# ml-unito/PartitionedLS.jl

Measured on AMD Instinct MI355X. Metric: sign-pattern NNLS solves/sec (whole node); fp64 obj gap vs ref, higher is better.
Workload: dtype f64

## Files before the change

### include/partls.h

```cpp
#ifndef PARTLS_H
#define PARTLS_H
#include <stdint.h>
#ifdef __cplusplus
extern "C" {
#endif

typedef enum {
    PARTLS_OK = 0,
    PARTLS_ERR_BAD_ARG = 1,
    PARTLS_ERR_BAD_PARTITION = 2,
    PARTLS_ERR_NONFINITE = 3,
    PARTLS_ERR_NO_DEVICE = 4,
    PARTLS_ERR_HIP = 5,
    PARTLS_ERR_NOT_CONVERGED = 6,
    PARTLS_ERR_UNSUPPORTED = 7,
    PARTLS_ERR_STATE = 8,
    PARTLS_ERR_ILL_CONDITIONED = 9
} partls_status;

#define PARTLS_OPT_FAITHFUL_INTERCEPT 1u
#define PARTLS_OPT_GENERIC_KERNEL     2u
#define PARTLS_OPT_RESCUE_CAPPED      4u

typedef struct partls_ctx partls_ctx;
// ... 105 lines not shown
partls_status partls_frontier_create(int n_groups, int rank, int world, int64_t batch, partls_frontier **out);
void          partls_frontier_destroy(partls_frontier *f);
partls_status partls_frontier_next(partls_frontier *f, int64_t *total, int64_t *mine, uint64_t *pat, uint64_t *free_groups,
                                   int32_t *src_slot, int32_t *per_rank);
partls_status partls_frontier_ingest(partls_frontier *f, const double *lb, const int32_t *branch, const int32_t *dst_slot,
                                     int32_t *dead, int64_t dead_capacity, int64_t *ndead);
partls_status partls_frontier_result(const partls_frontier *f, double *mu, uint64_t *pat, uint64_t *free_groups, int64_t *nodes);
partls_status partls_bnb_search(partls_ctx *ctx, int64_t max_nodes, double *mu, uint64_t *pat, uint64_t *free_groups, int64_t *nodes);

partls_status partls_predict(partls_ctx *ctx, const double *X, int64_t N, int64_t M, int64_t ldX,
                             const int64_t *P, int64_t K, int64_t ldP, const double *alpha, const double *beta, double t,
                             double *yhat);
partls_status partls_predict_device(partls_ctx *ctx, const double *dX, int64_t N, int64_t M, int64_t ldX,
                                    const int64_t *P, int64_t K, int64_t ldP, const double *alpha, const double *beta,
                                    double t, double *dyhat);


#define PARTLS_PREDICT_MANY_CHUNK 16
#define PARTLS_PREDICT_MANY_MAX_B 4096
#define PARTLS_PREDICT_MANY_BYTES (64ULL << 20)
partls_status partls_predict_many(partls_ctx *ctx, const double *X, int64_t N, int64_t M, int64_t ldX, int x_on_device,
                                  const int64_t *P, int64_t K, int64_t ldP, int64_t B, const double *alpha, const double *beta,
                                  const double *t, double *yhat, int64_t ldY, int64_t nr, const int64_t *ranks, double *stats,
                                  double *mean);

partls_status partls_synth_truth(uint64_t seed, int64_t D, int64_t K, int64_t *P, double *wstar);
partls_status partls_synth_device(partls_ctx *ctx, uint64_t seed, int64_t N, int64_t D, const double *wstar,
                                  double *dX, double *dy);

typedef enum {
    PARTLS_T_GRAM = 0,
    PARTLS_T_PREP = 1,
    PARTLS_T_SWEEP = 2,
    PARTLS_T_FINISH = 3,
    PARTLS_T_CALIB = 4,
    PARTLS_T_OOB = 5,
    PARTLS_T_RESCUE = 6,
    PARTLS_T_COUNT = 7
} partls_timer;
partls_status partls_get_timing(const partls_ctx *ctx, partls_timer which, double *ms);
partls_status partls_get_upload(const partls_ctx *ctx, double *ms, double *bytes);
partls_status partls_get_pivots(const partls_ctx *ctx, int64_t *pivots);
partls_status partls_get_vetoes(const partls_ctx *ctx, int64_t *vetoes);
partls_status partls_get_rescue_stats(const partls_ctx *ctx, int64_t *rescued, int64_t *pivots, int64_t *failed);
partls_status partls_get_blocks(const partls_ctx *ctx, int64_t *blocks);
partls_status partls_get_kkt_violation(const partls_ctx *ctx, double *violation, double *min_pivot);
typedef enum {
    PARTLS_ROUTE_REG_256 = 1,
    PARTLS_ROUTE_REG_512 = 2,
    PARTLS_ROUTE_DEFERRED = 3,
    PARTLS_ROUTE_EAGER = 4
} partls_route;
partls_status partls_get_sweep_route(const partls_ctx *ctx, int *kernel, int *tiles);
partls_status partls_get_near_ties(const partls_ctx *ctx, int64_t *evaluated);
partls_status partls_get_gram(const partls_ctx *ctx, double *G_aug);

#include "partls_f32.h"
#include "partls_f32_more.h"

#ifdef __cplusplus
}
#endif
#endif
```

### partitionedls.jl_amd/_lib.py

```python
import ctypes as C
import os
import subprocess

_HERE = os.path.dirname(os.path.abspath(__file__))
SO_PATH = os.environ.get("PARTLS_LIB") or os.path.join(_HERE, "libpartls_hip.so")
CSRC = os.path.join(_HERE, "csrc")

OK, ERR_BAD_ARG, ERR_BAD_PARTITION, ERR_NONFINITE, ERR_NO_DEVICE, ERR_HIP, ERR_NOT_CONVERGED, ERR_UNSUPPORTED, ERR_STATE, ERR_ILL_CONDITIONED = range(10)
OPT_FAITHFUL_INTERCEPT = 1
OPT_GENERIC_KERNEL = 2
OPT_RESCUE_CAPPED = 4
T_GRAM, T_PREP, T_SWEEP, T_FINISH, T_CALIB, T_OOB, T_RESCUE = range(7)
ROUTE_REG_256, ROUTE_REG_512, ROUTE_DEFERRED, ROUTE_EAGER = range(1, 5)
PREDICT_MANY_CHUNK, PREDICT_MANY_MAX_B, PREDICT_MANY_BYTES = 16, 4096, 64 << 20
OPT_TOP_MAX_K = 4096

_dp = C.POINTER(C.c_double)
_ip = C.POINTER(C.c_int64)
_i64 = C.c_int64

SYMBOLS = [
    ("partls_version", C.c_int, []),
    ("partls_last_error", C.c_char_p, []),
    ("partls_device_count", C.c_int, []),
# ... 21 lines not shown
    ("partls_opt_merge_candidates", C.c_int, [C.c_void_p, _i64, _dp, _ip, _dp, _ip]),
    ("partls_opt_pattern", C.c_int, [C.c_void_p, _i64, _dp, _dp]),
    ("partls_opt_models", C.c_int, [C.c_void_p, _i64, _i64, _ip, _dp, _dp, _i64, _dp, _i64, _dp, _i64, _dp, _ip, _ip]),
    ("partls_opt_top", C.c_int, [C.c_void_p, _i64, _i64, _i64, _ip, _dp, _dp, _i64, _dp, _i64, _dp, _i64, _dp, _ip, _ip, _ip]),
    ("partls_opt_top_select", C.c_int, [C.c_void_p, _dp, _i64, _i64, _i64, _ip, _ip, _dp, _ip]),
    ("partls_cv_opt", C.c_int, [C.c_void_p, C.c_void_p, _i64, _i64, _i64, C.c_void_p, C.c_int, C.c_void_p, _i64, _i64, _ip, _i64,
                                _dp, _i64, C.c_uint32, _dp, _i64, _dp, _i64, _dp, _dp, _ip, _dp, C.POINTER(C.c_int32)]),
    ("partls_cv_opt_weighted", C.c_int, [C.c_void_p, C.c_void_p, _i64, _i64, _i64, C.c_void_p, C.c_void_p, C.c_int, C.c_void_p, _i64,
                                         _i64, _ip, _i64, _dp, _i64, C.c_uint32, _dp, _i64, _dp, _i64, _dp, _dp, _ip, _dp,
                                         C.POINTER(C.c_int32)]),
    ("partls_opt_weightings", C.c_int, [C.c_void_p, C.c_void_p, _i64, _i64, _i64, C.c_void_p, C.c_int, C.c_void_p, _i64, _i64,
                                        C.c_void_p, _i64, _i64, C.c_double, C.c_uint32, _dp, _i64, _dp, _i64, _dp, _dp, _ip, _dp, _ip,
                                        C.POINTER(C.c_int32)]),
    ("partls_opt_num_patterns", _i64, [C.c_void_p]),
    ("partls_opt_bit_order", C.c_int, [C.c_void_p, _ip, _dp]),
    ("partls_fit_alt", C.c_int, [C.c_void_p, C.c_void_p, _i64, _i64, _i64, C.c_void_p, C.c_void_p, _i64, _i64, C.c_double,
                                 C.c_double, _i64, _dp, _dp, _dp, _dp, _dp, _dp, _ip]),
    ("partls_fit_bnb", C.c_int, [C.c_void_p, C.c_void_p, _i64, _i64, _i64, C.c_void_p, C.c_void_p, _i64, _i64, C.c_double,
                                 _dp, _dp, _dp, _dp, _ip]),
    ("partls_alt_prepared", C.c_int, [C.c_void_p, C.c_double, _i64, _dp, _dp, _dp, _dp, _dp, _dp, _ip]),
    ("partls_bnb_prepared", C.c_int, [C.c_void_p, _dp, _dp, _dp, _dp, _ip]),
    ("partls_alt_multistart", C.c_int, [C.c_void_p, C.c_double, _i64, _i64, _dp, _i64, _dp, _i64, _dp, _dp, _dp, _dp, _ip, _ip,
                                        _dp, _i64, _dp, _i64, _dp, _dp, _ip, C.POINTER(C.c_int32)]),
    ("partls_cv_alt", C.c_int, [C.c_void_p, C.c_void_p, _i64, _i64, _i64, C.c_void_p, C.c_void_p, C.c_int, C.c_void_p, _i64, _i64, _ip,
                                _i64, _dp, _i64, C.c_uint32, C.c_double, _i64, _i64, _dp, _i64, _dp, _i64,
                                _dp, _i64, _dp, _i64, _dp, _dp, _ip, _ip, _dp, C.POINTER(C.c_int32), _dp, _ip, C.POINTER(C.c_int32)]),
    ("partls_bnb_bound", C.c_int, [C.c_void_p, _i64, C.POINTER(C.c_uint64), C.POINTER(C.c_uint64), _dp, C.POINTER(C.c_int32)]),
    ("partls_bnb_snap_begin", C.c_int, [C.c_void_p]),
    ("partls_bnb_bound_snap", C.c_int, [C.c_void_p, _i64, C.POINTER(C.c_uint64), C.POINTER(C.c_uint64), C.POINTER(C.c_int32),
                                        C.POINTER(C.c_int32), _dp, C.POINTER(C.c_int32)]),
    ("partls_bnb_snap_release", C.c_int, [C.c_void_p, _i64, C.POINTER(C.c_int32)]),
    ("partls_frontier_create", C.c_int, [C.c_int, C.c_int, C.c_int, _i64, C.POINTER(C.c_void_p)]),
    ("partls_frontier_destroy", None, [C.c_void_p]),
    ("partls_frontier_next", C.c_int, [C.c_void_p, _ip, _ip, C.POINTER(C.c_uint64), C.POINTER(C.c_uint64), C.POINTER(C.c_int32),
                                       C.POINTER(C.c_int32)]),
    ("partls_frontier_ingest", C.c_int, [C.c_void_p, _dp, C.POINTER(C.c_int32), C.POINTER(C.c_int32), C.POINTER(C.c_int32), _i64, _ip]),
    ("partls_frontier_result", C.c_int, [C.c_void_p, _dp, C.POINTER(C.c_uint64), C.POINTER(C.c_uint64), _ip]),
    ("partls_bnb_search", C.c_int, [C.c_void_p, _i64, _dp, C.POINTER(C.c_uint64), C.POINTER(C.c_uint64), _ip]),
    ("partls_bnb_leaf", C.c_int, [C.c_void_p, C.c_uint64, C.c_uint64, _dp, _dp, _dp, _dp]),
    ("partls_predict", C.c_int, [C.c_void_p, C.c_void_p, _i64, _i64, _i64, C.c_void_p, _i64, _i64, _dp, _dp, C.c_double, _dp]),
    ("partls_predict_device", C.c_int, [C.c_void_p, C.c_void_p, _i64, _i64, _i64, C.c_void_p, _i64, _i64, _dp, _dp, C.c_double,
                                        C.c_void_p]),
    ("partls_predict_many", C.c_int, [C.c_void_p, C.c_void_p, _i64, _i64, _i64, C.c_int, C.c_void_p, _i64, _i64, _i64, _dp, _dp, _dp,
                                      C.c_void_p, _i64, _i64, _ip, C.c_void_p, C.c_void_p]),
    ("partls_synth_truth", C.c_int, [C.c_uint64, _i64, _i64, _ip, _dp]),
    ("partls_synth_device", C.c_int, [C.c_void_p, C.c_uint64, _i64, _i64, _dp, C.c_void_p, C.c_void_p]),
    ("partls_get_timing", C.c_int, [C.c_void_p, C.c_int, _dp]),
    ("partls_get_upload", C.c_int, [C.c_void_p, _dp, _dp]),
    ("partls_get_gram", C.c_int, [C.c_void_p, _dp]),
    ("partls_get_pivots", C.c_int, [C.c_void_p, _ip]),
    ("partls_get_vetoes", C.c_int, [C.c_void_p, _ip]),
    ("partls_get_rescue_stats", C.c_int, [C.c_void_p, _ip, _ip, _ip]),
    ("partls_get_blocks", C.c_int, [C.c_void_p, _ip]),
    ("partls_get_kkt_violation", C.c_int, [C.c_void_p, _dp, _dp]),
    ("partls_get_near_ties", C.c_int, [C.c_void_p, _ip]),
    ("partls_get_sweep_route", C.c_int, [C.c_void_p, C.POINTER(C.c_int), C.POINTER(C.c_int)]),
]

SYMBOLS_F32 = [
    ("partls_opt_prepare_f32", C.c_int, [C.c_void_p, C.c_void_p, _i64, _i64, _i64, C.c_void_p, C.c_void_p, C.c_int, C.c_void_p,
                                         _i64, _i64, C.c_double, C.c_uint32]),
    ("partls_predict_f32", C.c_int, [C.c_void_p, C.c_void_p, _i64, _i64, _i64, C.c_void_p, _i64, _i64, _dp, _dp, C.c_double, _dp]),
    ("partls_predict_device_f32", C.c_int, [C.c_void_p, C.c_void_p, _i64, _i64, _i64, C.c_void_p, _i64, _i64, _dp, _dp, C.c_double,
                                            C.c_void_p]),
]

SYMBOLS_F32_MORE = [
    ("partls_predict_many_f32", C.c_int, [C.c_void_p, C.c_void_p, _i64, _i64, _i64, C.c_int, C.c_void_p, _i64, _i64, _i64, _dp, _dp, _dp,
                                          C.c_void_p, _i64, _i64, _ip, C.c_void_p, C.c_void_p]),
]

_lib = None


def build(force=False):
    args = ["make", "-C", CSRC, "-s", "-j8"]
    if force:
        args.append("-B")
    subprocess.check_call(args)
    return SO_PATH


def _preload_torch_hip_runtime():
    import importlib.util
    import sys
    if "torch" in sys.modules:
        return
    if os.environ.get("PARTLS_NO_TORCH_RUNTIME"):
        return
    try:
        spec = importlib.util.find_spec("torch")
    except Exception:
        spec = None
    if spec is None or not spec.origin:
        return
    cand = os.path.join(os.path.dirname(spec.origin), "lib", "libamdhip64.so")
    if os.path.exists(cand):
        try:
            C.CDLL(cand, mode=C.RTLD_GLOBAL)
        except OSError:
            pass


def lib():
    global _lib
    if _lib is None:
# ... 14 lines not shown
```

### partitionedls.jl_amd/api.py

```python
import atexit
import ctypes as C
import warnings
import weakref
from contextlib import contextmanager
from dataclasses import dataclass
from typing import NamedTuple

import numpy as np

from . import _lib as L


class PartlsError(RuntimeError):
    def __init__(self, status, msg):
        super().__init__(f"partls status {status}: {msg}")
        self.status = status


class Opt:
    """Optimal algorithm: complete enumeration of the sign patterns."""


class Alt:
    """Alternating optimisation."""
# ... 488 lines not shown
        B = a.shape[0]
        yh = np.zeros((N, B), order="F") if want_yhat else None
        st = None if r is None else np.zeros((N, len(r)), order="F")
        mu = np.zeros(N) if want_mean else None
        self._predict_many(X.ctypes.data, 0, X.dtype == np.float32, N, M, N, P, a, b, tv, None if yh is None else yh.ctypes.data, N, r,
                           None if st is None else st.ctypes.data, None if mu is None else mu.ctypes.data)
        return dict(yhat=yh, stats=st, mean=mu)

    def predict_many_device(self, dX_ptr, N, M, ldX, P, alpha, beta, t, *, dyhat_ptr=None, ldY=0, ranks=None, dstats_ptr=None,
                            dmean_ptr=None, dtype=np.float64):
        f32 = _f32(dtype, "predict_many_device")
        P = np.asfortranarray(P, dtype=np.int64)
        a, b, tv, r = _many_models(alpha, beta, t, int(M), P.shape[1], ranks)
        if (r is None) != (dstats_ptr is None):
            raise ValueError("predict_many_device: dstats_ptr goes with ranks")
        self._predict_many(C.c_void_p(dX_ptr), 1, f32, int(N), int(M), int(ldX), P, a, b, tv,
                           None if dyhat_ptr is None else C.c_void_p(dyhat_ptr), int(ldY), r,
                           None if dstats_ptr is None else C.c_void_p(dstats_ptr), None if dmean_ptr is None else C.c_void_p(dmean_ptr))

    def _predict_many(self, xp, on_device, f32, N, M, ldX, P, a, b, tv, yhat, ldY, ranks, stats, mean):
        lib = L.lib()
        fn = lib.partls_predict_many_f32 if f32 else lib.partls_predict_many
        _check(fn(self._h, xp, N, M, ldX, on_device, P.ctypes.data, P.shape[1], M, a.shape[0], _dp(a), _dp(b), _dp(tv), yhat, ldY,
                  0 if ranks is None else len(ranks), None if ranks is None else _ip(ranks), stats, mean))

    def _count(self, getter):
        n = C.c_int64()
        _check(getter(self._h, C.byref(n)))
        return n.value

    def timing(self, which):
        ms = C.c_double()
        _check(L.lib().partls_get_timing(self._h, int(which), C.byref(ms)))
        return ms.value

    def upload(self):
        ms = C.c_double(); b = C.c_double()
        _check(L.lib().partls_get_upload(self._h, C.byref(ms), C.byref(b)))
        return ms.value, b.value

    def pivots(self):
        return self._count(L.lib().partls_get_pivots)

    def vetoes(self):
        return self._count(L.lib().partls_get_vetoes)

    def rescue_stats(self):
        r = C.c_int64(); p = C.c_int64(); f = C.c_int64()
        _check(L.lib().partls_get_rescue_stats(self._h, C.byref(r), C.byref(p), C.byref(f)))
        return Report(rescued=r.value, pivots=p.value, failed=f.value)

    def blocks(self):
        return self._count(L.lib().partls_get_blocks)

    def sweep_route(self):
        k = C.c_int(); t = C.c_int()
        _check(L.lib().partls_get_sweep_route(self._h, C.byref(k), C.byref(t)))
        return k.value, t.value

    def kkt_violation(self):
        v = C.c_double()
        _check(L.lib().partls_get_kkt_violation(self._h, C.byref(v), None))
        return v.value

    def min_pivot(self):
        v = C.c_double(); mp = C.c_double()
        _check(L.lib().partls_get_kkt_violation(self._h, C.byref(v), C.byref(mp)))
        return mp.value

    def gram(self):
        N, M, K = self._shape
        G = np.zeros((M + 2, M + 2), order="F")
        _check(L.lib().partls_get_gram(self._h, _dp(G)))
        return G

    def synth_device(self, seed, N, D, wstar, dX_ptr, dy_ptr):
        ws = np.ascontiguousarray(wstar, dtype=np.float64)
        _check(L.lib().partls_synth_device(self._h, C.c_uint64(seed), N, D, _dp(ws), C.c_void_p(dX_ptr), C.c_void_p(dy_ptr)))


class Frontier:

    def __init__(self, n_groups, rank=0, world=1, batch=1024):
        self._h = C.c_void_p()
        _check(L.lib().partls_frontier_create(int(n_groups), int(rank), int(world), int(batch), C.byref(self._h)))
        self.world, self.batch = int(world), int(batch)
        self._pat = np.zeros(self.batch, dtype=np.uint64); self._free = np.zeros(self.batch, dtype=np.uint64)
        self._src = np.zeros(self.batch, dtype=np.int32); self._per = np.zeros(self.world, dtype=np.int32)
        self._dead = np.zeros(4 * self.batch * self.world + 64, dtype=np.int32)

    def close(self):
        if self._h:
            L.lib().partls_frontier_destroy(self._h)
            self._h = C.c_void_p()

    def __del__(self):
        try:
            self.close()
        except Exception:
            pass

    def next(self):
        tot = C.c_int64(); mine = C.c_int64()
        _check(L.lib().partls_frontier_next(self._h, C.byref(tot), C.byref(mine), _u64p(self._pat), _u64p(self._free), _i32p(self._src),
                                            _i32p(self._per)))
        m = mine.value
# ... 750 lines not shown
```

### partitionedls.jl_amd/csrc/api.hip

```cpp
#include "ctx.h"
#include <cstdarg>
#include <cstdio>
#include <cstdlib>
#include <cstring>
#include <new>

namespace partls {

static thread_local char g_err[512] = "";
static thread_local bool g_runtime_gone = false;
bool runtime_gone() { return g_runtime_gone; }
void set_error(const char *fmt, ...)
{
    va_list ap;
    va_start(ap, fmt);
    vsnprintf(g_err, sizeof(g_err), fmt, ap);
    va_end(ap);
}

void t_begin(partls_ctx *c, int w) { (void)hipEventRecord(c->ev0[w], c->stream); }
void t_end(partls_ctx *c, int w) { (void)hipEventRecord(c->ev1[w], c->stream); c->timed[w] = true; }
void t_collect(partls_ctx *c)
{
    for (int w = 0; w < PARTLS_T_COUNT; ++w)
// ... 24 lines not shown
}

partls_status predict_weights(const int64_t *P, int64_t M, int64_t K, int64_t ldP, const double *alpha, const double *beta, double *w)
{
    for (int64_t m = 0; m < M; ++m) {
        double s = 0.0;
        for (int64_t k = 0; k < K; ++k) {
            const int64_t v = P[m + k * ldP];
            if (v != 0 && v != 1) { set_error("P has an entry outside {0,1}"); return PARTLS_ERR_BAD_PARTITION; }
            s += (double)v * alpha[m] * beta[k];
        }
        w[m] = s;
    }
    return PARTLS_OK;
}

}

using namespace partls;

extern "C" {

int partls_version(void) { return 106; }
const char *partls_last_error(void) { return g_err; }

int partls_device_count(void)
{
    int n = 0;
    if (hipGetDeviceCount(&n) != hipSuccess) return 0;
    return n;
}

partls_status partls_create(int device, partls_ctx **out)
try {
    if (!out) { set_error("partls_create: out is NULL"); return PARTLS_ERR_BAD_ARG; }
    *out = nullptr;
    int n = partls_device_count();
    if (n <= 0 || device < 0 || device >= n) {
        set_error("partls_create: no usable HIP device (count=%d, requested=%d); this library has no CPU fallback", n, device);
        return PARTLS_ERR_NO_DEVICE;
    }
    PARTLS_HIP_CHECK(hipSetDevice(device));
    partls_ctx *c = new (std::nothrow) partls_ctx();
    if (!c) { set_error("out of host memory"); return PARTLS_ERR_BAD_ARG; }
    c->device = device;
    if (hipDeviceGetAttribute(&c->ncu, hipDeviceAttributeMultiprocessorCount, device) != hipSuccess || c->ncu < 1) c->ncu = 256;
    if (const char *e = getenv("PARTLS_TOL_REL")) c->knobs.tol_rel = atof(e);
    if (const char *e = getenv("PARTLS_CHAIN_LEN")) c->knobs.chain_len = atoll(e);
    if (const char *e = getenv("PARTLS_GRID")) c->knobs.grid = atoll(e);
    if (const char *e = getenv("PARTLS_GRAM_S")) c->knobs.gram_S = atoi(e);
    if (const char *e = getenv("PARTLS_GRAM_CR")) c->knobs.gram_cr = atoi(e);
    if (const char *e = getenv("PARTLS_COOP_ROWS")) c->knobs.coop_rows = atoi(e);
    if (const char *e = getenv("PARTLS_PAIR")) c->knobs.pair = atoi(e) != 0 ? 1 : 0;
    if (const char *e = getenv("PARTLS_BIT_ORDER")) c->knobs.bit_order = !strcmp(e, "identity") ? 1 : (!strcmp(e, "calibrate") ? 2 : 0);
    if (const char *e = getenv("PARTLS_ALT_MS_MAX_ROUNDS")) c->knobs.alt_ms_max_rounds = atoi(e);
    if (const char *e = getenv("PARTLS_MAX_ROUNDS")) { const int v = atoi(e); if (v >= 1) c->knobs.max_rounds = v; }
    if (const char *e = getenv("PARTLS_RESCUE_MAX_PASSES")) { const int v = atoi(e); if (v >= 1) c->knobs.rescue_max_passes = v; }
    if (const char *e = getenv("PARTLS_ALT_MS_CHUNK")) c->knobs.alt_ms_chunk = atoll(e);
    if (const char *e = getenv("PARTLS_TOP_PIECE")) c->knobs.top_piece = atoll(e);
    if (const char *e = getenv("PARTLS_BATCH_PIECE")) c->knobs.batch_piece = atoi(e);
    if (const char *e = getenv("PARTLS_KKT_TOL")) c->knobs.kkt_tol = atof(e);
    if (const char *e = getenv("PARTLS_NEAR_TIE_REL")) c->knobs.near_tie_rel = atof(e);
    if (const char *e = getenv("PARTLS_CAL_WB")) c->knobs.cal_wb = atof(e);
    if (const char *e = getenv("PARTLS_CAL_WS")) c->knobs.cal_ws = atof(e);
    c->knobs.no_coop = getenv("PARTLS_NO_COOP") != nullptr;
    c->knobs.no_export = getenv("PARTLS_NO_EXPORT") != nullptr;
    c->knobs.no_staged_upload = getenv("PARTLS_NO_STAGED_UPLOAD") != nullptr;
    if (const char *e = getenv("PARTLS_REG_MAXT")) { const int v = atoi(e); if (v >= 1 && v <= 20) c->knobs.reg_maxt = v; }
    c->knobs.eager_generic = getenv("PARTLS_EAGER_GENERIC") != nullptr;
    c->knobs.bnb_cold = getenv("PARTLS_BNB_COLD") != nullptr;
    if (const char *e = getenv("PARTLS_BNB_BATCH")) c->knobs.bnb_batch = atoi(e);
    if (const char *e = getenv("PARTLS_BNB_POOL_MB")) c->knobs.bnb_pool_mb = atoi(e);
    if (const char *e = getenv("PARTLS_BNB_WG_PER_CU")) c->knobs.bnb_wg_per_cu = atoi(e);
    if (const char *e = getenv("PARTLS_COOP_FAULT")) c->knobs.coop_fault = atoi(e);
    c->knobs.lz_fault = getenv("PARTLS_LZ_FAULT") != nullptr;
    c->knobs.no_tab_refine = getenv("PARTLS_NO_TAB_REFINE") != nullptr;
    c->knobs.finish_trace = getenv("PARTLS_FINISH_TRACE") != nullptr;
    c->knobs.alt_trace = getenv("PARTLS_ALT_TRACE") != nullptr;
    c->knobs.alt_always_check = getenv("PARTLS_ALT_ALWAYS_CHECK") != nullptr;
    c->knobs.print_stamps = getenv("PARTLS_PRINT_STAMPS") != nullptr;
    c->knobs.cv_serial = getenv("PARTLS_CV_SERIAL") != nullptr && strcmp(getenv("PARTLS_CV_SERIAL"), "0") != 0;
    c->knobs.resample_serial = getenv("PARTLS_RESAMPLE_SERIAL") != nullptr && strcmp(getenv("PARTLS_RESAMPLE_SERIAL"), "0") != 0;
    hipError_t e = hipStreamCreateWithFlags(&c->stream, hipStreamNonBlocking);
    for (int w = 0; w < PARTLS_T_COUNT && e == hipSuccess; ++w) {
        e = hipEventCreate(&c->ev0[w]);
        if (e == hipSuccess) e = hipEventCreate(&c->ev1[w]);
    }
    if (e != hipSuccess) {
        set_error("partls_create: stream / event creation failed: %s", hipGetErrorString(e));
        partls_destroy(c);
        return PARTLS_ERR_HIP;
    }
    *out = c;
    return PARTLS_OK;
}
PARTLS_ABI_GUARD

void partls_destroy(partls_ctx *c)
{
    if (!c) return;
    partls_destroy(c->cv_work);
    for (partls_ctx *v : c->cv_view) partls_destroy(v);
    c->cv_work = nullptr;
    c->cv_view.clear();
    int ndev = 0;
    const bool alive = hipGetDeviceCount(&ndev) == hipSuccess && ndev > c->device && hipSetDevice(c->device) == hipSuccess;
// ... 116 lines not shown
PARTLS_ABI_GUARD

partls_status partls_get_upload(const partls_ctx *c, double *ms, double *bytes)
try {
    if (!c || !ms || !bytes) { set_error("partls_get_upload: bad argument"); return PARTLS_ERR_BAD_ARG; }
    *ms = c->last_upload_ms; *bytes = c->last_upload_bytes;
    return PARTLS_OK;
}
PARTLS_ABI_GUARD

partls_status partls_get_pivots(const partls_ctx *c, int64_t *pivots)
try {
    if (!c || !pivots) { set_error("partls_get_pivots: bad argument"); return PARTLS_ERR_BAD_ARG; }
    *pivots = (int64_t)c->last_pivots;
    return PARTLS_OK;
}
PARTLS_ABI_GUARD

partls_status partls_get_kkt_violation(const partls_ctx *c, double *violation, double *min_pivot)
try {
    if (!c || !violation) { set_error("partls_get_kkt_violation: bad argument"); return PARTLS_ERR_BAD_ARG; }
    *violation = c->last_kkt;
    if (min_pivot) *min_pivot = c->last_min_loo;
    return PARTLS_OK;
}
PARTLS_ABI_GUARD

partls_status partls_get_rescue_stats(const partls_ctx *c, int64_t *rescued, int64_t *pivots, int64_t *failed)
try {
    if (!c) { set_error("partls_get_rescue_stats: bad argument"); return PARTLS_ERR_BAD_ARG; }
    if (rescued) *rescued = (int64_t)c->rescue_rescued;
    if (pivots) *pivots = (int64_t)c->rescue_pivots;
    if (failed) *failed = (int64_t)c->rescue_failed;
    return PARTLS_OK;
}
PARTLS_ABI_GUARD

partls_status partls_get_vetoes(const partls_ctx *c, int64_t *vetoes)
try {
    if (!c || !vetoes) { set_error("partls_get_vetoes: bad argument"); return PARTLS_ERR_BAD_ARG; }
    *vetoes = (int64_t)c->last_vetoes;
    return PARTLS_OK;
}
PARTLS_ABI_GUARD

partls_status partls_get_blocks(const partls_ctx *c, int64_t *blocks)
try {
    if (!c || !blocks) { set_error("partls_get_blocks: bad argument"); return PARTLS_ERR_BAD_ARG; }
    *blocks = (int64_t)c->last_blocks;
    return PARTLS_OK;
}
PARTLS_ABI_GUARD

partls_status partls_get_sweep_route(const partls_ctx *c, int *kernel, int *tiles)
try {
    if (!c || !kernel || !tiles) { set_error("partls_get_sweep_route: bad argument"); return PARTLS_ERR_BAD_ARG; }
    const partls_ctx *p = c->prepared ? c : (c->cv_work && c->cv_work->prepared ? c->cv_work : nullptr);
    if (!p) { set_error("partls_get_sweep_route: context not prepared"); return PARTLS_ERR_STATE; }
    *kernel = p->use_reg ? (sweep_reg_small(p->T) ? PARTLS_ROUTE_REG_256 : PARTLS_ROUTE_REG_512)
                         : (p->knobs.eager_generic ? PARTLS_ROUTE_EAGER : PARTLS_ROUTE_DEFERRED);
    *tiles = p->use_reg ? p->T : 0;
    return PARTLS_OK;
}
PARTLS_ABI_GUARD

partls_status partls_get_near_ties(const partls_ctx *c, int64_t *evaluated)
try {
    if (!c || !evaluated) { set_error("partls_get_near_ties: bad argument"); return PARTLS_ERR_BAD_ARG; }
    *evaluated = c->last_near_evaluated;
    return PARTLS_OK;
}
PARTLS_ABI_GUARD

partls_status partls_get_gram(const partls_ctx *c, double *G_aug)
try {
    if (!c || !c->prepared || !G_aug) { set_error("partls_get_gram: context not prepared"); return PARTLS_ERR_STATE; }
    const int na = (int)c->M + 2;
    for (int j = 0; j < na; ++j)
        for (int i = 0; i < na; ++i) G_aug[(size_t)i + (size_t)j * na] = h_reg(c, i, j);
    return PARTLS_OK;
}
PARTLS_ABI_GUARD

}
```

### partitionedls.jl_amd/csrc/ctx.h

```cpp
#pragma once
#include "common.h"
#include <chrono>
#include <functional>
#include <vector>

namespace partls {

bool runtime_gone();
struct NoCopy {
    NoCopy() = default;
    NoCopy(const NoCopy &) = delete;
    NoCopy &operator=(const NoCopy &) = delete;
};

struct DevBuf : NoCopy {
    void *p = nullptr;
    size_t bytes = 0;
    ~DevBuf() { release(); }
    hipError_t ensure(size_t b)
    {
        if (b <= bytes && p) return hipSuccess;
        if (p) { hipError_t e = hipFree(p); p = nullptr; bytes = 0; if (e != hipSuccess) return e; }
        hipError_t e = hipMalloc(&p, b ? b : 8);
        if (e == hipSuccess) bytes = b;
// ... 46 lines not shown
        if (e != hipSuccess) p = nullptr;
        return e;
    }
    void release() { if (p && !runtime_gone()) (void)hipHostFree(p); p = nullptr; }
    operator T *() const { return p; }
};

struct UploadStaging : NoCopy {
    char *pin[8] = {};
    hipStream_t stream[4] = {};
    hipEvent_t event[8] = {};
    ~UploadStaging()
    {
        if (runtime_gone()) return;
        for (int i = 0; i < 8; ++i) { if (pin[i]) (void)hipHostFree(pin[i]); if (event[i]) (void)hipEventDestroy(event[i]); }
        for (int t = 0; t < 4; ++t) if (stream[t]) (void)hipStreamDestroy(stream[t]);
    }
};

}

struct partls_knobs {
    double tol_rel = 1e-11;
    long long chain_len = 0;
    long long grid = 0;
    int gram_S = 0, gram_cr = 0;
    int coop_rows = 0;
    bool no_coop = false;
    int reg_maxt = 18;
    bool no_staged_upload = false;
    bool no_export = false;
    bool eager_generic = false;
    int bnb_batch = 1024;
    int bnb_pool_mb = 65536;
    int bnb_wg_per_cu = 8;
    bool bnb_cold = false;
    bool lz_fault = false;
    int coop_fault = 0;
    bool no_tab_refine = false;
    bool finish_trace = false;
    bool alt_trace = false;
    bool alt_always_check = false;
    bool print_stamps = false;
    int alt_ms_max_rounds = 0;
    int max_rounds = 0;
    int rescue_max_passes = 0;
    long long alt_ms_chunk = 0;
    double kkt_tol = 1e-12;
    double near_tie_rel = 1e-13;
    double cal_wb = 1.0, cal_ws = 1.0;
    bool cv_serial = false;
    bool resample_serial = false;
    int pair = -1;
    long long top_piece = 0;
    int bit_order = 0;
    int batch_piece = 0;
};

struct partls_ctx {
    int device = 0;
    int ncu = 256;
    partls_knobs knobs;
    hipStream_t stream = nullptr;
    hipEvent_t ev0[PARTLS_T_COUNT] = {}, ev1[PARTLS_T_COUNT] = {};
    bool timed[PARTLS_T_COUNT] = {};
    double ms[PARTLS_T_COUNT] = {};

    bool prepared = false;
    int64_t N = 0, M = 0, K = 0, ldX = 0;
    double eta = 0.0;
    uint32_t flags = 0;
    bool faithful = false;
    const void *dX = nullptr;
    bool x_f32 = false;
    const double *dy = nullptr;
    partls::DevBuf ownX, ownY;
    const double *dw = nullptr, *ds = nullptr;
    partls::DevBuf ownW, ownS, wPart;
    bool multi_rank = false;
    std::vector<int64_t> P;
    std::vector<uint64_t> mask_aug;
    std::vector<uint64_t> pack;
    const uint64_t *maskTabP = nullptr;
    const int *permP = nullptr;
    int ldg = 0, chunks = 0;
    partls::DevBuf slab, G, maskAugD , scale, Tfull, T0reg, scratch, bestObj, bestSol , bestPat, counters, allOpt,
        wdev, partial, yhatD, gD, nodeCode, nodeSol, nodeObj, predX, predY, gridCtr, nodeTab, nodeBasic, altA, altGA, altHg,
        nodePiv, maskInt, allOptRef, bnbIn, bnbOut, altGersh, amsState, amsWork;
    partls::DevChunks bnbChunks;
    size_t bnbSlotBytes = 0, bnbMaxSlots = 0;
    int bnbChunkSlots = 512;
    std::vector<int> bnbFree, bnbRefs;
    std::vector<partls_ctx *> peers;
    partls::PinnedDoubles hPart, hGpart;
    partls::PinnedDoubles sweepOut, nodeOut, exportSol;
    partls::DevBuf mdlRows, mdlOut, mdlCtr;
    partls::PinnedDoubles mdlStage;
    partls::DevBuf topWork, topRows;
    partls::DevBuf rescueScratch, rescueList;
    partls::PinnedDoubles rescueStage;
    unsigned long long rescue_rescued = 0, rescue_pivots = 0, rescue_failed = 0;
    std::function<partls_status(partls_ctx *)> gram_hook;
    partls::PinnedDoubles amsHostIn, amsHostOut;
    partls::PinnedDoubles bnbHostIn, bnbHostOut;
    partls::UploadStaging up;
    double last_upload_ms = 0.0, last_upload_bytes = 0.0;
// ... 180 lines not shown
```

### partitionedls.jl_amd/csrc/sweep_setup.hip

```cpp
#include "ctx.h"
#include "near_tie.h"
#include "sweep_rules.h"
#include <algorithm>
#include <cmath>
#include <cstring>
#include <numeric>

namespace partls {

SweepParams sweep_params(const partls_ctx *c, bool internal_order)
{
    SweepParams p{};
    const bool permuted = internal_order && !c->order_identity;
    p.n = c->n; p.kbits = c->kbits;
    p.mask = permuted ? c->maskInt.as<uint64_t>() : c->maskTabP;
    p.scratch = c->scratch.as<double>();
    p.tol = c->tol; p.piv_eps = SWEEP_PIV_EPS; p.max_rounds = c->knobs.max_rounds >= 1 ? c->knobs.max_rounds : sweep_max_rounds(c->n);
    for (int k = 0; k < 40; ++k) p.rbit.gbit[k] = (uint8_t)k;
    if (permuted) for (int k = 0; k < c->kbits; ++k) p.rbit.gbit[c->order.gbit[k]] = (uint8_t)k;
    return p;
}

partls_status ensure_sweep_scratch(partls_ctx *c, int grid)
{
    const size_t ld = (size_t)c->n + 1;
    PARTLS_HIP_CHECK(c->scratch.ensure((c->use_reg ? 64 : (size_t)grid * ld * ld) * sizeof(double)));
    return PARTLS_OK;
}

partls_status node_sweep_params(partls_ctx *c, size_t nodes, int64_t chain_len, int grid, SweepParams *p)
{
    const size_t wgs = (size_t)std::max(grid, 4096);
    PARTLS_HIP_CHECK(c->bestObj.ensure(sizeof(double) * wgs));
    PARTLS_HIP_CHECK(c->bestPat.ensure(sizeof(int64_t) * wgs));
    *p = sweep_params(c, false);
    p->g_begin = 0; p->g_end = (int64_t)nodes; p->chain_len = chain_len;
    p->best_obj = c->bestObj.as<double>(); p->best_pat = c->bestPat.as<int64_t>();
    return PARTLS_OK;
}

void bind_sweep_block(SweepParams &p, double *base, int grid, bool runner_up)
{
    const SweepBlock b = sweep_block(base, grid, runner_up);
    bind_counters(p, b.counters);
    p.best_obj = b.best_obj; p.best_pat = b.best_pat;
    p.second_obj = b.second_obj; p.second_pat = b.second_pat;
}

hipError_t launch_any_sweep(partls_ctx *c, SweepParams &p, int grid, bool models)
{
    if (c->use_reg) {
        p.T0 = c->T0reg.as<double>();
        return launch_sweep_blk(p, c->T, grid, c->stream, models);
    }
    p.T0 = c->Tfull.as<double>();
// ... 208 lines not shown
    c->flip_cost = cost;
    double pred_ref = 0.0, pred_sorted = 0.0, wgt = 0.5;
    for (int b = 0; b < kb; ++b, wgt *= 0.5) { pred_ref += wgt * cost[(size_t)b]; pred_sorted += wgt * cost[(size_t)by_cost[(size_t)b]]; }
    if (c->knobs.bit_order != 2 && !(pred_sorted < 0.98 * pred_ref)) return PARTLS_OK;
    bool ident = true;
    for (int b = 0; b < kb; ++b) { c->order.gbit[by_cost[(size_t)b]] = (uint8_t)b; ident = ident && by_cost[(size_t)b] == b; }
    if (ident) return PARTLS_OK;
    std::vector<uint64_t> mi((size_t)n);
    for (int i = 0; i < n; ++i) {
        uint64_t m = c->mask_tab[(size_t)i], q = 0;
        for (; m; m &= m - 1) q |= 1ULL << c->order.gbit[__builtin_ctzll(m)];
        mi[(size_t)i] = q;
    }
    PARTLS_HIP_CHECK(c->maskInt.ensure((size_t)n * sizeof(uint64_t)));
    PARTLS_HIP_CHECK(hipMemcpyAsync(c->maskInt.p, mi.data(), (size_t)n * sizeof(uint64_t), hipMemcpyHostToDevice, c->stream));
    PARTLS_HIP_CHECK(hipStreamSynchronize(c->stream));
    c->order_identity = false;
    return PARTLS_OK;
}

int64_t partls::reference_pattern(const partls_ctx *c, int64_t q)
{
    if (q < 0 || c->order_identity) return q;
    uint64_t r = 0;
    for (int k = 0; k < c->kbits; ++k) r |= (((uint64_t)q >> c->order.gbit[k]) & 1ULL) << k;
    return (int64_t)r;
}

static bool on_bit0(const partls_ctx *c, int i)
{
    if (c->hScale[(size_t)i] == 0.0) return false;
    for (int k = 0; k < c->kbits; ++k)
        if (c->order.gbit[k] == 0 && ((c->mask_tab[(size_t)i] >> k) & 1ULL)) return true;
    return false;
}

static bool pair_rule(const partls_ctx *c, int64_t total)
{
    if (!c->use_reg || sweep_reg_small(c->T) || c->T > 16 || c->knobs.pair == 0) return false;
    int live = 0;
    for (int i = 0; i < c->n; ++i) live += on_bit0(c, i);
    if (live > 16) return false;
    if (c->knobs.pair == 1) return true;
    const int kb = c->kbits, seg_len = (kb + (kb >= 8 ? 2 : 1) - 1) / (kb >= 8 ? 2 : 1);
    if (kb < 2 || ((int64_t)1 << kb) < (int64_t)c->ncu * 32 * (8 + seg_len) || total < (int64_t)c->ncu * 32) return false;
    return live >= 12;
}

bool partls::sweep_pairs(const partls_ctx *c, int64_t total) { return c->pair_laid && pair_rule(c, total); }

partls_status partls::pair_relayout(partls_ctx *c)
{
    if (c->pair_laid || !pair_rule(c, (int64_t)1 << c->kbits)) return PARTLS_OK;
    const int n = c->n, base = 16 * (c->T - 2);
    std::vector<int> grp, oth, idx;
    for (int i = 0; i < n; ++i) (on_bit0(c, i) ? grp : oth).push_back(i);
    idx.assign(oth.begin(), oth.begin() + base);
    idx.insert(idx.end(), grp.begin(), grp.end());
    idx.insert(idx.end(), oth.begin() + base, oth.end());
    c->pair_laid = true;
    bool same = true;
    for (int i = 0; i < n; ++i) same = same && idx[(size_t)i] == i;
    if (same) return PARTLS_OK;
    std::vector<int> perm((size_t)n);
    std::vector<double> sc((size_t)n);
    for (int i = 0; i < n; ++i) { perm[(size_t)i] = c->perm[(size_t)idx[(size_t)i]]; sc[(size_t)i] = c->hScale[(size_t)idx[(size_t)i]]; }
    c->perm = perm;
    std::memcpy(c->hScale.data(), sc.data(), (size_t)n * sizeof(double));
    const partls_status st = ctx_layout_tableau(c, false);
    if (st != PARTLS_OK) return st;
    if (!c->order_identity) {
        c->mask_int_host.resize((size_t)n);
        for (int i = 0; i < n; ++i) {
            uint64_t m = c->mask_tab[(size_t)i], q = 0;
            for (; m; m &= m - 1) q |= 1ULL << c->order.gbit[__builtin_ctzll(m)];
            c->mask_int_host[(size_t)i] = q;
        }
        PARTLS_HIP_CHECK(hipMemcpyAsync(c->maskInt.p, c->mask_int_host.data(), (size_t)n * sizeof(uint64_t), hipMemcpyHostToDevice, c->stream));
    }
    c->coop_state_valid = false;
    c->tab_valid = false;
    return PARTLS_OK;
}

partls_status partls::prepare_sweep_order(partls_ctx *c)
{
    const partls_status st = calibrate_bit_order(c);
    return st != PARTLS_OK ? st : pair_relayout(c);
}

bool partls::sweep_plan(partls_ctx *c, int64_t total, int64_t *chain_len_out, int *grid_out, const char *who)
{
    int64_t chain_len;
    if (c->knobs.chain_len > 0) chain_len = c->knobs.chain_len;
    else if (c->use_reg) {
        const int ncu = c->ncu;
        const int64_t per_chain = total >= (int64_t)ncu * 2048 * 8 ? 2048 : 1024;
        const int conc = sweep_reg_concurrency(c->T);
        if (conc > 1) {
            const int64_t slots = (int64_t)ncu * conc;
            const int64_t k = std::max<int64_t>(1, (total + slots * per_chain - 1) / (slots * per_chain));
            chain_len = std::max<int64_t>(4, (total + k * slots - 1) / (k * slots));
        } else {
        int64_t k = (total + (int64_t)ncu * per_chain - 1) / ((int64_t)ncu * per_chain);
        if (k < 2) k = 2;
        chain_len = (total + k * ncu - 1) / (k * ncu);
        if (chain_len < 16) chain_len = 16;
        }
    } else {
        const int ncu = c->ncu;
        chain_len = 256;
        while (chain_len > 16 && (total + chain_len - 1) / chain_len < ncu) chain_len >>= 1;
// ... 46 lines not shown
```

Baseline: 24.95 million.

## Align tableau column layout to Gray-walk bit groups in pair relayout

Measured after the change: 25.17 million (median of 6 runs). Within noise of the previous version (+0.9%).

```diff
diff --git a/include/partls.h b/include/partls.h
--- a/include/partls.h
+++ b/include/partls.h
@@ -181,6 +181,7 @@
     PARTLS_ROUTE_EAGER = 4
 } partls_route;
 partls_status partls_get_sweep_route(const partls_ctx *ctx, int *kernel, int *tiles);
+int partls_get_tableau_order(const partls_ctx *ctx, int32_t *feature_of_slot, int cap);
 partls_status partls_get_near_ties(const partls_ctx *ctx, int64_t *evaluated);
 partls_status partls_get_gram(const partls_ctx *ctx, double *G_aug);
 
diff --git a/partitionedls.jl_amd/_lib.py b/partitionedls.jl_amd/_lib.py
--- a/partitionedls.jl_amd/_lib.py
+++ b/partitionedls.jl_amd/_lib.py
@@ -97,6 +97,7 @@
     ("partls_get_vetoes", C.c_int, [C.c_void_p, _ip]),
     ("partls_get_rescue_stats", C.c_int, [C.c_void_p, _ip, _ip, _ip]),
     ("partls_get_blocks", C.c_int, [C.c_void_p, _ip]),
+    ("partls_get_tableau_order", C.c_int, [C.c_void_p, C.POINTER(C.c_int32), C.c_int]),
     ("partls_get_kkt_violation", C.c_int, [C.c_void_p, _dp, _dp]),
     ("partls_get_near_ties", C.c_int, [C.c_void_p, _ip]),
     ("partls_get_sweep_route", C.c_int, [C.c_void_p, C.POINTER(C.c_int), C.POINTER(C.c_int)]),
diff --git a/partitionedls.jl_amd/api.py b/partitionedls.jl_amd/api.py
--- a/partitionedls.jl_amd/api.py
+++ b/partitionedls.jl_amd/api.py
@@ -564,6 +564,13 @@
 
     def blocks(self):
         return self._count(L.lib().partls_get_blocks)
+
+    def tableau_order(self):
+        fn = L.lib().partls_get_tableau_order
+        out = np.zeros(max(int(fn(self._h, None, 0)), 0), dtype=np.int32)
+        if len(out):
+            fn(self._h, out.ctypes.data_as(C.POINTER(C.c_int32)), len(out))
+        return out
 
     def sweep_route(self):
         k = C.c_int(); t = C.c_int()
diff --git a/partitionedls.jl_amd/csrc/api.hip b/partitionedls.jl_amd/csrc/api.hip
--- a/partitionedls.jl_amd/csrc/api.hip
+++ b/partitionedls.jl_amd/csrc/api.hip
@@ -100,6 +100,7 @@
     if (const char *e = getenv("PARTLS_GRAM_CR")) c->knobs.gram_cr = atoi(e);
     if (const char *e = getenv("PARTLS_COOP_ROWS")) c->knobs.coop_rows = atoi(e);
     if (const char *e = getenv("PARTLS_PAIR")) c->knobs.pair = atoi(e) != 0 ? 1 : 0;
+    if (const char *e = getenv("PARTLS_WALK_LAYOUT")) c->knobs.walk_layout = atoi(e) != 0;
     if (const char *e = getenv("PARTLS_BIT_ORDER")) c->knobs.bit_order = !strcmp(e, "identity") ? 1 : (!strcmp(e, "calibrate") ? 2 : 0);
     if (const char *e = getenv("PARTLS_ALT_MS_MAX_ROUNDS")) c->knobs.alt_ms_max_rounds = atoi(e);
     if (const char *e = getenv("PARTLS_MAX_ROUNDS")) { const int v = atoi(e); if (v >= 1) c->knobs.max_rounds = v; }
@@ -322,6 +323,14 @@
 }
 PARTLS_ABI_GUARD
 
+int partls_get_tableau_order(const partls_ctx *c, int32_t *feature_of_slot, int cap)
+{
+    if (!c || !c->prepared || (cap > 0 && !feature_of_slot)) return 0;
+    const int n = (size_t)c->n <= c->perm.size() ? c->n : (int)c->perm.size();
+    for (int s = 0; s < n && s < cap; ++s) feature_of_slot[s] = (int32_t)c->perm[(size_t)s];
+    return n;
+}
+
 partls_status partls_get_sweep_route(const partls_ctx *c, int *kernel, int *tiles)
 try {
     if (!c || !kernel || !tiles) { set_error("partls_get_sweep_route: bad argument"); return PARTLS_ERR_BAD_ARG; }
diff --git a/partitionedls.jl_amd/csrc/ctx.h b/partitionedls.jl_amd/csrc/ctx.h
--- a/partitionedls.jl_amd/csrc/ctx.h
+++ b/partitionedls.jl_amd/csrc/ctx.h
@@ -122,6 +122,7 @@
     bool cv_serial = false;
     bool resample_serial = false;
     int pair = -1;
+    bool walk_layout = true;
     long long top_piece = 0;
     int bit_order = 0;
     int batch_piece = 0;
diff --git a/partitionedls.jl_amd/csrc/sweep_setup.hip b/partitionedls.jl_amd/csrc/sweep_setup.hip
--- a/partitionedls.jl_amd/csrc/sweep_setup.hip
+++ b/partitionedls.jl_amd/csrc/sweep_setup.hip
@@ -1,6 +1,7 @@
 #include "ctx.h"
 #include "near_tie.h"
 #include "sweep_rules.h"
+#include "walk_layout.h"
 #include <algorithm>
 #include <cmath>
 #include <cstring>
@@ -315,12 +316,15 @@
 partls_status partls::pair_relayout(partls_ctx *c)
 {
     if (c->pair_laid || !pair_rule(c, (int64_t)1 << c->kbits)) return PARTLS_OK;
-    const int n = c->n, base = 16 * (c->T - 2);
-    std::vector<int> grp, oth, idx;
-    for (int i = 0; i < n; ++i) (on_bit0(c, i) ? grp : oth).push_back(i);
-    idx.assign(oth.begin(), oth.begin() + base);
-    idx.insert(idx.end(), grp.begin(), grp.end());
-    idx.insert(idx.end(), oth.begin() + base, oth.end());
+    const int n = c->n;
+    std::vector<uint8_t> live((size_t)n);
+    std::vector<int> bit((size_t)n, -1);
+    for (int i = 0; i < n; ++i) {
+        live[(size_t)i] = c->hScale[(size_t)i] != 0.0;
+        for (int k = 0; k < c->kbits; ++k)
+            if (((c->mask_tab[(size_t)i] >> k) & 1ULL) && (bit[(size_t)i] < 0 || c->order.gbit[k] < bit[(size_t)i])) bit[(size_t)i] = c->order.gbit[k];
+    }
+    const std::vector<int> idx = walk_layout(n, c->T, live.data(), bit.data(), c->knobs.walk_layout).idx;
     c->pair_laid = true;
     bool same = true;
     for (int i = 0; i < n; ++i) same = same && idx[(size_t)i] == i;
diff --git a/partitionedls.jl_amd/csrc/walk_layout.h b/partitionedls.jl_amd/csrc/walk_layout.h
--- /dev/null
+++ b/partitionedls.jl_amd/csrc/walk_layout.h
@@ -0,0 +1,90 @@
+#pragma once
+#include <cstddef>
+#include <cstdint>
+#include <vector>
+
+namespace partls {
+
+static constexpr int WALK_LAYOUT_W = 16;
+static constexpr int WALK_LAYOUT_MB = 8;
+
+inline double walk_layout_cost(int n, int T, const uint8_t *live, const int *bit, const int *idx)
+{
+    std::vector<int> cnt((size_t)64 * (size_t)T, 0);
+    for (int s = 0; s < n; ++s) {
+        const int i = idx[s];
+        if (live[i] && bit[i] >= 0 && bit[i] < 64) ++cnt[(size_t)bit[i] * (size_t)T + (size_t)(s / WALK_LAYOUT_W)];
+    }
+    double cost = 0.0, wgt = 1.0;
+    for (int b = 0; b < 64; ++b, wgt *= 0.5) {
+        int blocks = 0;
+        for (int t = 0; t < T; ++t) blocks += (cnt[(size_t)b * (size_t)T + (size_t)t] + WALK_LAYOUT_MB - 1) / WALK_LAYOUT_MB;
+        cost += wgt * blocks;
+    }
+    return cost;
+}
+
+inline void walk_layout_plain(int n, int T, const uint8_t *live, const int *bit, int *idx)
+{
+    const int base = WALK_LAYOUT_W * (T - 2);
+    std::vector<int> grp, oth;
+    for (int i = 0; i < n; ++i) (live[i] && bit[i] == 0 ? grp : oth).push_back(i);
+    int s = 0;
+    if (base > (int)oth.size()) grp.clear(), oth.clear();
+    for (int o = 0; o < base && o < (int)oth.size(); ++o) idx[s++] = oth[(size_t)o];
+    for (int i : grp) idx[s++] = i;
+    for (int o = base; o < (int)oth.size(); ++o) idx[s++] = oth[(size_t)o];
+    for (; s < n; ++s) idx[s] = s;
+}
+
+struct WalkLayout {
+    std::vector<int> idx;
+    double cost_plain = 0.0;
+    double cost_aligned = 0.0;
+    int placed = 0;
+    bool aligned = false;
+};
+
+inline WalkLayout walk_layout(int n, int T, const uint8_t *live, const int *bit, bool align = true)
+{
+    constexpr int W = WALK_LAYOUT_W;
+    WalkLayout out;
+    out.idx.resize((size_t)(n > 0 ? n : 0));
+    for (int i = 0; i < n; ++i) out.idx[(size_t)i] = i;
+    int g0 = 0;
+    for (int i = 0; i < n; ++i) g0 += live[i] && bit[i] == 0;
+    if (n < 1 || T < 2 || n <= W * (T - 1) || n > W * T || g0 > W) return out;
+
+    std::vector<int> plain((size_t)n), slot((size_t)n, -1);
+    walk_layout_plain(n, T, live, bit, plain.data());
+    std::vector<char> taken((size_t)n, 0);
+    std::vector<int> fill((size_t)T, 0);
+    auto put = [&](int col, int b) {
+        for (int i = 0; i < n; ++i)
+            if (live[i] && bit[i] == b) { slot[(size_t)(W * col + fill[(size_t)col]++)] = i; taken[(size_t)i] = 1; }
+    };
+    put(T - 2, 0);
+    for (int b = 1; b < 64; ++b) {
+        int s = 0;
+        for (int i = 0; i < n; ++i) s += live[i] && bit[i] == b;
+        if (s == 0 || s > W) continue;
+        int col = 0;
+        while (col < T - 2 && W - fill[(size_t)col] < s) ++col;
+        if (col >= T - 2) break;
+        put(col, b);
+        ++out.placed;
+    }
+    int s = 0;
+    for (int i = 0; i < n; ++i) {
+        if (taken[(size_t)i]) continue;
+        while (slot[(size_t)s] >= 0) ++s;
+        slot[(size_t)s++] = i;
+    }
+    out.cost_plain = walk_layout_cost(n, T, live, bit, plain.data());
+    out.cost_aligned = walk_layout_cost(n, T, live, bit, slot.data());
+    out.aligned = align && out.cost_aligned <= out.cost_plain;
+    out.idx = out.aligned ? slot : plain;
+    return out;
+}
+
+}
```
